# NVIDIA-ISAAC-ROS/isaac_ros_nvblox

Hardware: NVIDIA H100
Metric: depth-frames/sec (TSDF+ESDF integrate, 640x480 @ 5 cm voxels) (higher is better)
Workload: dtype f32

## Files before the change

### isaac_ros_nvblox_b200/csrc/nvb_api.cu

```cuda
#include <algorithm>
#include <array>
#include <cfloat>
#include <cmath>
#include <cstdio>
#include <cstring>
#include <set>
#include <string>
#include <vector>

#include "nvb_internal.cuh"

using namespace nvb;

namespace {

thread_local std::string g_last_error;

int fail(int code, const std::string& msg) {
  g_last_error = msg;
  return code;
}

#define NVB_CUDA(expr)                                                                               \
  do {                                                                                               \
// ... 315 lines not shown
  N.count = L->count;
  N.free_count = L->free_count;
  NVB_CUDA(cudaMalloc(&N.free_slots, (size_t)new_capacity * sizeof(int)));
  NVB_CUDA(cudaMemcpyAsync(N.free_slots, L->free_slots, (size_t)L->capacity * sizeof(int), cudaMemcpyDeviceToDevice,
                           m->stream));
  N.capacity = new_capacity;
  N.block_bytes = L->block_bytes;
  NVB_CUDA(cudaMalloc(&N.blocks, (size_t)new_capacity * L->block_bytes));
  NVB_CUDA(cudaMemsetAsync(N.blocks, 0, (size_t)new_capacity * L->block_bytes, m->stream));
  NVB_CUDA(cudaMemcpyAsync(N.blocks, L->blocks, (size_t)count * L->block_bytes, cudaMemcpyDeviceToDevice, m->stream));
  NVB_CUDA(cudaMalloc(&N.block_index, (size_t)new_capacity * 3 * sizeof(int)));
  NVB_CUDA(cudaMemcpyAsync(N.block_index, L->block_index, (size_t)count * 3 * sizeof(int), cudaMemcpyDeviceToDevice,
                           m->stream));
  const int hcap = nextPow2(2ll * new_capacity);
  N.hash.mask = (unsigned int)hcap - 1;
  NVB_CUDA(cudaMalloc(&N.hash.keys, (size_t)hcap * sizeof(unsigned long long)));
  NVB_CUDA(cudaMalloc(&N.hash.vals, (size_t)hcap * sizeof(int)));
  launchFillU64(N.hash.keys, kEmptyKey, (size_t)hcap, m->stream);
  launchRehash(N, count, m->stream);
  NVB_CUDA(syncAll(m));
  cudaFree(L->blocks), cudaFree(L->block_index), cudaFree(L->hash.keys), cudaFree(L->hash.vals), cudaFree(L->free_slots);
  *L = N;
  return NVB_OK;
}

int allocWaveXRecords(NvbMapper* m, int cap) {
  const int grid = esdfWaveXGrid(m->num_sms, m->esdf_reserved_sms);
  NVB_CUDA(syncAll(m));
  if (m->xrec) cudaFree(m->xrec);
  m->xrec = nullptr;
  m->xseg = 6 * ((cap + grid - 1) / grid) + 64;
  m->xseg_grid = grid;
  NVB_CUDA(cudaMalloc(&m->xrec, 2 * (size_t)grid * m->xseg * 32 * sizeof(int)));
  return NVB_OK;
}

int allocEsdfScratch(NvbMapper* m, int old_cap, int cap) {
  int rc;
  if ((rc = reallocCopy(&m->work, 0, (size_t)cap, false, m->stream))) return rc;
  if ((rc = reallocCopy(&m->upd_list, 0, (size_t)cap, false, m->stream))) return rc;
  if ((rc = reallocCopy(&m->clr_list, 0, (size_t)cap, false, m->stream))) return rc;
  if ((rc = reallocCopy(&m->clr_cand, 0, (size_t)cap, false, m->stream))) return rc;
  if ((rc = reallocCopy(&m->cleared_list, (size_t)old_cap, (size_t)cap, true, m->stream))) return rc;
  if ((rc = reallocCopy(&m->ring_a, 0, (size_t)cap, false, m->stream))) return rc;
  if ((rc = reallocCopy(&m->ring_b, 0, (size_t)cap, false, m->stream))) return rc;
  if ((rc = reallocCopy(&m->stamp_a, (size_t)old_cap, (size_t)cap, true, m->stream))) return rc;
  if ((rc = reallocCopy(&m->stamp_b, (size_t)old_cap, (size_t)cap, true, m->stream))) return rc;
  if ((rc = reallocCopy(&m->seed_upd, (size_t)old_cap, (size_t)cap, true, m->stream))) return rc;
  if ((rc = reallocCopy(&m->seed_clr, (size_t)old_cap, (size_t)cap, true, m->stream))) return rc;
  if ((rc = reallocCopy(&m->psum, 2 * (size_t)old_cap, 2 * (size_t)cap, true, m->stream))) return rc;
  {
    int* q = nullptr;
    NVB_CUDA(cudaMalloc(&q, (size_t)cap * 6 * sizeof(int)));
    NVB_CUDA(cudaMemsetAsync(q, 0xFE, (size_t)cap * 6 * sizeof(int), m->stream));
    if (m->nbr && old_cap)
      NVB_CUDA(cudaMemcpyAsync(q, m->nbr, (size_t)old_cap * 6 * sizeof(int), cudaMemcpyDeviceToDevice, m->stream));
    NVB_CUDA(syncAll(m));
    if (m->nbr) cudaFree(m->nbr);
    m->nbr = q;
  }
  {
    int* q = nullptr;
    NVB_CUDA(cudaMalloc(&q, (size_t)cap * 27 * sizeof(int)));
    NVB_CUDA(cudaMemsetAsync(q, 0xFE, (size_t)cap * 27 * sizeof(int), m->stream));
    if (m->nbr27 && old_cap)
      NVB_CUDA(cudaMemcpyAsync(q, m->nbr27, (size_t)old_cap * 27 * sizeof(int), cudaMemcpyDeviceToDevice, m->stream));
    NVB_CUDA(syncAll(m));
    if (m->nbr27) cudaFree(m->nbr27);
    m->nbr27 = q;
  }
  if ((rc = reallocCopy(&m->cand_stamp, (size_t)old_cap, (size_t)cap, true, m->stream))) return rc;
  if ((rc = reallocCopy(&m->cand_a, 0, (size_t)cap, false, m->stream))) return rc;
  if ((rc = reallocCopy(&m->cand_b, 0, (size_t)cap, false, m->stream))) return rc;
  if (m->esdf_persistent == 2) {
    if (m->shadow) cudaFree(m->shadow);
    m->shadow = nullptr;
    NVB_CUDA(cudaMalloc(&m->shadow, (size_t)cap * kEsdfBlockBytes));
    m->shadow_cap = cap;
  }
  if (m->esdf_persistent == 3) {
    NVB_CUDA(syncAll(m));
    if (m->xslab) cudaFree(m->xslab);
    m->xslab = nullptr;
    NVB_CUDA(cudaMalloc(&m->xslab, 2 * (size_t)cap * kEsdfBlockBytes));
    int rc;
    if ((rc = allocWaveXRecords(m, cap))) return rc;
    if (!m->xcounts) {
      NVB_CUDA(cudaMalloc(&m->xcounts, esdfWaveXFlagBytes()));
      NVB_CUDA(cudaMemsetAsync(m->xcounts, 0, esdfWaveXFlagBytes(), m->stream));
    }
  }
  return NVB_OK;
}

int allocTsdfSide(NvbMapper* m, int old_cap, int cap) {
  int rc;
  if ((rc = reallocCopy(&m->dirty, (size_t)old_cap, (size_t)cap, true, m->stream))) return rc;
  if ((rc = reallocCopy(&m->todo_slots, (size_t)old_cap, (size_t)cap, true, m->stream))) return rc;
  if (m->projective_layer_type == NVB_PROJECTIVE_TSDF_WITH_FREESPACE) {
    if ((rc = reallocCopy(&m->dirty_fs, (size_t)old_cap, (size_t)cap, true, m->stream))) return rc;
    if ((rc = reallocCopy(&m->todo_fs_slots, (size_t)old_cap, (size_t)cap, true, m->stream))) return rc;
  }
  if (m->dirty_mesh) {
    if ((rc = reallocCopy(&m->dirty_mesh, (size_t)old_cap, (size_t)cap, true, m->stream))) return rc;
    if ((rc = reallocCopy(&m->todo_mesh_slots, (size_t)old_cap, (size_t)cap, true, m->stream))) return rc;
  }
  return NVB_OK;
}

constexpr int kHostListCap = 1 << 15;

enum { kWorkCount = 0, kUpdCount = 1, kClrCount = 2, kClrAabb = 3, kClearedCount = 9, kRingCount = 10, kRingId = 14,
       kTodoCount = 15, kFrameCount = 16, kError = 17, kClearedSeq = 18, kTailState = 20, kDeadCount = 22, kDeadClearedCount = 23, kGesCounts = 24, kTodoFsCount = 28, kFsWorkCount = 29, kColsCount = 30, kColorWorkCount = 31, kXTail = 32, kTodoMeshCount = 36, kClrCandCount = 37, kNumInts = 40 };

float logOddsFromProbability(float p);

EsdfCtx makeEsdfCtx(NvbMapper* m) {
  EsdfCtx c{};
  c.tsdf = m->tsdf, c.esdf = m->esdf;
  c.freespace = m->freespace;
  c.use_freespace = m->projective_layer_type == NVB_PROJECTIVE_TSDF_WITH_FREESPACE ? 1 : 0;
  c.work = m->work;
  c.work_count = m->esdf_ints + kWorkCount;
  c.upd_list = m->upd_list, c.upd_count = m->esdf_ints + kUpdCount;
  c.clr_list = m->clr_list, c.clr_count = m->esdf_ints + kClrCount;
  c.clr_cand = m->clr_cand, c.clr_cand_count = m->esdf_ints + kClrCandCount;
  c.clr_aabb = m->esdf_ints + kClrAabb;
  c.cleared_list = m->cleared_list, c.cleared_count = m->esdf_ints + kClearedCount;
  c.ring_a = m->ring_a, c.ring_b = m->ring_b;
  c.ring_count = m->esdf_ints + kRingCount;
  c.tail_state = m->esdf_ints + kTailState;
  c.stamp_a = m->stamp_a, c.stamp_b = m->stamp_b;
  c.ring_id = m->esdf_ints + kRingId;
  c.nbr = m->nbr, c.seed_upd = m->seed_upd, c.seed_clr = m->seed_clr;
  c.clr_bits = m->clr_bits;
  c.psum = m->psum, c.prune = (m->prune_ok && m->esdf_persistent == 3) ? 1 : 0;
  c.nbr27 = m->nbr27, c.shadow = m->shadow, c.cand_stamp = m->cand_stamp;
  c.xslab = m->xslab, c.xrec = m->xrec, c.xtail = m->esdf_ints + kXTail, c.xseg = m->xseg, c.xcounts = m->xcounts;
  c.xsplit_min_k = m->esdf_split_min_k;
  c.ges_counts = m->esdf_ints + kGesCounts;
  c.cand_a = m->cand_a, c.cand_b = m->cand_b, c.ges_switch = m->ges_switch;
  c.colset_keys = m->colset, c.colset_mask = m->colset_n ? (unsigned int)(m->colset_n - 1) : 0u;
  c.cols = m->cols, c.cols_count = m->esdf_ints + kColsCount;
  c.dead_cleared_xyz = m->dead_cleared_xyz;
  c.dead_cleared_count = m->dead_cleared_xyz ? m->esdf_ints + kDeadClearedCount : nullptr;
  c.cleared_seq = m->esdf_ints + kClearedSeq;
  c.update_seq = m->update_seq;
  c.barrier = m->barrier;
  c.phase_max = m->phase_max;
  c.stats = m->stats;
  c.error = m->error_dev;
  const float max_esdf_distance_vox = m->ep.max_esdf_distance_m / m->voxel_size;
  c.max_sq = max_esdf_distance_vox * max_esdf_distance_vox;
  c.max_esdf_distance_m = m->ep.max_esdf_distance_m;
  c.max_site_distance_m = m->ep.max_site_distance_vox * m->voxel_size;
  c.min_weight = m->ep.min_weight;
  c.block_size = m->block_size;
  c.from_occupancy = m->projective_layer_type == NVB_PROJECTIVE_OCCUPANCY ? 1 : 0;
  c.occupied_threshold_log_odds = logOddsFromProbability(m->ep.occupied_threshold);
  return c;
}

float logOddsFromProbability(float p) {
  p = fmaxf(1e-3f, fminf(p, 1.0f - 1e-3f));
  return logf(p / (1.0f - p));
}

// ... 2987 lines not shown
```

### isaac_ros_nvblox_b200/csrc/nvb_esdf_wavex.cu

```cuda
#include "nvb_esdf_wave_common.cuh"

#include <cstdlib>

namespace nvb {

namespace {

#ifndef NVB_WAVEX_THREADS
#define NVB_WAVEX_THREADS 512
#endif
#ifndef NVB_WAVEX_MAXREG
#define NVB_WAVEX_MAXREG 96
#endif
#ifndef NVB_WAVEX_TAIL
#define NVB_WAVEX_TAIL 1
#endif
#ifndef NVB_WAVEX_PROF
#define NVB_WAVEX_PROF 0
#endif
#ifndef NVB_WAVEX_SPEC_HALO
#define NVB_WAVEX_SPEC_HALO 0
#endif
#if NVB_WAVEX_PROF
#define X_PROF_BEGIN() long long tq = clock64();
#define X_PROF(i) \
  if (lane64 == 0) xs.prof[group][i] += clock64() - tq; \
  tq = clock64();
#define X_PROF_COUNT(i) \
  if (lane64 == 0) xs.prof[group][i]++;
#define X_PROF_BIN(i, j, K)                                                  \
  if (lane64 == 0) {                                                         \
    const int kb = (K) <= 256 ? 0 : ((K) <= 1040 ? 1 : 2);                   \
    const long long dt = clock64() - tq;                                     \
    xs.prof[group][i] += dt, xs.prof[group][(j) + kb] += dt, xs.prof[group][(j) + 3 + kb]++; \
  }                                                                          \
  tq = clock64();
#else
#define X_PROF_BEGIN()
#define X_PROF(i)
#define X_PROF_COUNT(i)
#define X_PROF_BIN(i, j, K)
#endif
constexpr int kXT = NVB_WAVEX_THREADS;
constexpr int kXG = kXT / 64;
constexpr int kRecInts = 32;
constexpr int kMaxCtas = 192;
constexpr int kRX = 110, kRY = 11;
constexpr int kRegionVox = 1100;
constexpr int kFlagBase = 4 * kRegionVox;
constexpr int kXRegionWords = 5 * kRegionVox;
constexpr size_t kXSmemBytes = (size_t)kXG * kXRegionWords * sizeof(unsigned int);

struct XTables {
  unsigned int halo[8][64];
  unsigned int pair[6][4][64];
};

struct XShared {
  int rec[kXG][kRecInts];
  int nb[kXG][8];
  int pos[kXG][8];
  unsigned int mask[kXG];
  int changed[kXG];
  unsigned int live[kXG][8];
  int seg[kXG][2];
  int pre[kMaxCtas + 1];
  int warp_tot[2][8];
  int ncand, nchanged;
  int next;
  int cur[kXG];
  int seeds[kXG];
  int bcast[4];
  unsigned int generation;
  int n_bar;
  int ring;
  int swept, faces, rings, n_tail;
  int n_split, n_rest;
#if NVB_WAVEX_PROF
  long long prof[kXG][16];
#endif
};

struct XCtx {
  unsigned char* blocks;
  int* block_index;
  DevHash hash;
  int* nbr;
  int* nbr27;
  int* cand_stamp;
  unsigned int* psum;
  int* stamp[2];
  unsigned char* X[2];
  int* recs[2];
  int seg;
  int split_min_k;
  int* error;
  float max_sq;
  __device__ __forceinline__ int* segment(int p, int cta) const { return recs[p] + (size_t)cta * seg * kRecInts; }
};

__shared__ XTables x_tab;
__shared__ XShared x_xs;
__shared__ XCtx x_ctx;
extern __shared__ __align__(16) unsigned int x_smem[];

__device__ __forceinline__ int rvox(int rx, int ry, int rz) { return rx * kRX + ry * kRY + rz; }
__device__ __forceinline__ int faceEntry(int f) {
  return f == 0 ? 22 : (f == 1 ? 4 : (f == 2 ? 16 : (f == 3 ? 10 : (f == 4 ? 14 : 12))));
}
__device__ __forceinline__ int boundaryOff(int r) { return r == 0 ? -1 : (r == 9 ? 1 : 0); }
__device__ __forceinline__ int boundaryLoc(int r) { return r == 0 ? 7 : (r == 9 ? 0 : r - 1); }

__device__ __forceinline__ int neighbor27(const XCtx& c, int slot, int d) {
  int v = __ldcg(c.nbr27 + 27 * slot + d);
  if (v < -1) {
    const int* bi = c.block_index + 3 * slot;
    v = (d == 13) ? slot : hashFind(c.hash, bi[0] + d / 9 - 1, bi[1] + (d / 3) % 3 - 1, bi[2] + d % 3 - 1);
    c.nbr27[27 * slot + d] = v;
  }
  return v;
}
__device__ __forceinline__ int neighbor6(const XCtx& c, int slot, int dir) {
  int v = __ldcg(c.nbr + 6 * slot + dir);
  if (v < -1) {
    const int* bi = c.block_index + 3 * slot;
    const int d = (dir & 1) ? -1 : 1;
    v = hashFind(c.hash, bi[0] + ((dir >> 1) == 0 ? d : 0), bi[1] + ((dir >> 1) == 1 ? d : 0), bi[2] + ((dir >> 1) == 2 ? d : 0));
    c.nbr[6 * slot + dir] = v;
  }
  return v;
}

__device__ __forceinline__ void initTables(XTables& tab, int tid) {
  for (int i = tid; i < 512; i += kXT) {
    const int k = i >> 6, lane = i & 63;
    unsigned int e = 0;
    int ra = 1, r1 = 1, r2 = 1, axis = 0;
    bool valid = true;
    if (k < 6) {
      axis = k >> 1;
      ra = (k & 1) ? 0 : 9, r1 = (lane >> 3) + 1, r2 = (lane & 7) + 1;
    } else {
      const int n = i - 384;
      if (n < 96) {
        const int edge = n >> 3, cn = edge & 3;
        axis = edge >> 2;
        ra = (n & 7) + 1, r1 = (cn & 1) ? 9 : 0, r2 = (cn & 2) ? 9 : 0;
      } else if (n < 104) {
        const int cn = n - 96;
        ra = (cn & 1) ? 9 : 0, r1 = (cn & 2) ? 9 : 0, r2 = (cn & 4) ? 9 : 0;
      } else {
        valid = false;
      }
    }
    if (valid) {
      const int rx = axis == 0 ? ra : r1, ry = axis == 0 ? r1 : (axis == 1 ? ra : r2), rz = axis == 2 ? ra : r2;
      const int d = (boundaryOff(rx) + 1) * 9 + (boundaryOff(ry) + 1) * 3 + (boundaryOff(rz) + 1);
      e = (unsigned)rvox(rx, ry, rz) | ((unsigned)(boundaryLoc(rx) * 64 + boundaryLoc(ry) * 8 + boundaryLoc(rz)) << 11) |
          ((unsigned)d << 20) | (1u << 25);
    }
    tab.halo[k][lane] = e;
  }
  for (int i = tid; i < 6 * 4 * 64; i += kXT) {
    const int pass = i >> 8, j = (i >> 6) & 3, lane = i & 63;
    const int axis = pass >> 1, dir = (pass & 1) ? -1 : 1;
    int plane, u, w;
    bool valid = true;
    if (j < 2) {
      plane = j, u = (lane >> 3) + 1, w = (lane & 7) + 1;
    } else {
      const int n = (j - 2) * 64 + lane;
      plane = n / 36;
      const int q = n % 36;
      if (q < 10) u = 0, w = q;
      else if (q < 20) u = 9, w = q - 10;
      else if (q < 28) u = q - 20 + 1, w = 0;
      else u = q - 28 + 1, w = 9;
      if (n >= 72) valid = false, plane = 0, u = 1, w = 1;
    }
    unsigned int e = 0;
    if (valid) {
      const int sa = dir > 0 ? (plane ? 8 : 0) : (plane ? 9 : 1);
      const int so = dir > 0 ? (plane ? 0 : -1) : (plane ? 1 : 0);
      const int da = sa + dir;
      const int A = axis == 0 ? 9 : (axis == 1 ? 3 : 1), U = axis == 0 ? 3 : 9, W = axis == 2 ? 3 : 1;
      const int d = 13 + so * A + boundaryOff(u) * U + boundaryOff(w) * W;
      const int inner = da >= 1 && da <= 8 && u >= 1 && u <= 8 && w >= 1 && w <= 8;
      const int sv = axis == 0 ? rvox(sa, u, w) : (axis == 1 ? rvox(u, sa, w) : rvox(u, w, sa));
      const int dv = axis == 0 ? rvox(da, u, w) : (axis == 1 ? rvox(u, da, w) : rvox(u, w, da));
      e = (unsigned)sv | ((unsigned)dv << 11) | ((unsigned)d << 22) | ((unsigned)inner << 27) | (1u << 28);
    }
    tab.pair[pass][j][lane] = e;
  }
}

struct LiveMasks {
  unsigned int* live;
  unsigned int needed;
  unsigned int axes;
};
__device__ __forceinline__ LiveMasks liveMasks(unsigned int mask, unsigned int* live_smem, bool writer) {
  LiveMasks L;
  L.live = live_smem;
  const unsigned int ok = mask | (1u << 13);
  const unsigned int D[6] = {0x7FFFE00u, 0x3FE00u, 0x3F000u, 0x7000u, 0x6000u, 0x2000u};
  unsigned int acc = 0;
  L.axes = 0;
#pragma unroll
  for (int p = 0; p < 6; p++) {
    const int axis = p >> 1;
    const int A = axis == 0 ? 9 : (axis == 1 ? 3 : 1);
    const unsigned int lo = axis == 0 ? 0x000001ffu : (axis == 1 ? 0x001c0e07u : 0x01249249u);
    const unsigned int dst_ok = ok & D[p];
    unsigned int lv, dst;
    if ((p & 1) == 0) {
      lv = mask & (lo | (lo << A)) & (dst_ok >> A);
      dst = lv << A;
    } else {
      lv = mask & ((lo << A) | (lo << (2 * A))) & (dst_ok << A);
      dst = lv >> A;
    }
    if (writer) live_smem[p] = lv;
    if (lv) L.axes |= 1u << axis;
    acc |= lv | dst;
  }
  L.needed = acc & mask & ~(1u << 13);
  return L;
}

struct OwnRegs {
  uint4 q[10];
};
__device__ __forceinline__ OwnRegs ownLoad(const unsigned char* blk, int lane64) {
  OwnRegs o;
  const uint4* src = reinterpret_cast<const uint4*>(blk) + lane64 * 10;
#pragma unroll
  for (int i = 0; i < 10; i++) o.q[i] = __ldcg(src + i);
  return o;
}
__device__ __forceinline__ unsigned int liveAxes(const unsigned int* live) {
  return ((live[0] | live[1]) ? 1u : 0u) | ((live[2] | live[3]) ? 2u : 0u) | ((live[4] | live[5]) ? 4u : 0u);
}
__device__ __forceinline__ unsigned int ownWord(const OwnRegs& o, int w) {
  const uint4& v = o.q[w >> 2];
  return (w & 3) == 0 ? v.x : ((w & 3) == 1 ? v.y : ((w & 3) == 2 ? v.z : v.w));
}
__device__ __forceinline__ void ownToShared(unsigned int* R, const OwnRegs& o, int lane64) {
  uint4* A = reinterpret_cast<uint4*>(R);
  const int v0 = rvox((lane64 >> 3) + 1, (lane64 & 7) + 1, 1);
#pragma unroll
  for (int z = 0; z < 8; z++) {
    A[v0 + z] = make_uint4(ownWord(o, 5 * z), ownWord(o, 5 * z + 1), ownWord(o, 5 * z + 2), ownWord(o, 5 * z + 3));
    R[kFlagBase + v0 + z] = ownWord(o, 5 * z + 4);
  }
}
__device__ __forceinline__ void ownStore(unsigned char* layer_blk, bool to_layer, unsigned char* x_blk, const unsigned int* R,
                                         unsigned int* psum_slot, int lane64) {
  const uint4* A = reinterpret_cast<const uint4*>(R);
  const int x = lane64 >> 3, y = lane64 & 7;
  const int v0 = rvox(x + 1, y + 1, 1);
  uint4* dl = reinterpret_cast<uint4*>(layer_blk) + lane64 * 10;
  uint4* dx = reinterpret_cast<uint4*>(x_blk) + lane64 * 10;
  int lo0 = 99, lo1 = 99, lo2 = 99, hi0 = -99, hi1 = -99, hi2 = -99;
#pragma unroll
  for (int h = 0; h < 2; h++) {
    unsigned int w[20];
#pragma unroll
    for (int z = 0; z < 4; z++) {
      const uint4 a = A[v0 + 4 * h + z];
      w[5 * z] = a.x, w[5 * z + 1] = a.y, w[5 * z + 2] = a.z, w[5 * z + 3] = a.w;
      w[5 * z + 4] = R[kFlagBase + v0 + 4 * h + z];
      if ((a.y | a.z | a.w) != 0u) {
        const int b0 = (x + (int)a.y) >> 3, b1 = (y + (int)a.z) >> 3, b2 = (4 * h + z + (int)a.w) >> 3;
        lo0 = min(lo0, b0), hi0 = max(hi0, b0), lo1 = min(lo1, b1), hi1 = max(hi1, b1), lo2 = min(lo2, b2), hi2 = max(hi2, b2);
      }
    }
#pragma unroll
    for (int i = 0; i < 5; i++) {
      const uint4 v = make_uint4(w[4 * i], w[4 * i + 1], w[4 * i + 2], w[4 * i + 3]);
      if (to_layer) __stcg(dl + 5 * h + i, v);
      __stcg(dx + 5 * h + i, v);
    }
  }
  if (psum_slot) {
    lo0 = __reduce_min_sync(0xffffffffu, lo0), lo1 = __reduce_min_sync(0xffffffffu, lo1), lo2 = __reduce_min_sync(0xffffffffu, lo2);
    hi0 = __reduce_max_sync(0xffffffffu, hi0), hi1 = __reduce_max_sync(0xffffffffu, hi1), hi2 = __reduce_max_sync(0xffffffffu, hi2);
    if ((lane64 & 31) == 0) {
      unsigned int v = 0u;
      if (lo0 <= hi0) {
        const bool fits = lo0 >= -16 && lo1 >= -16 && lo2 >= -16 && hi0 <= 15 && hi1 <= 15 && hi2 <= 15;
        v = fits ? ((1u << 31) | (unsigned)(lo0 + 16) | ((unsigned)(hi0 + 16) << 5) | ((unsigned)(lo1 + 16) << 10) |
                    ((unsigned)(hi1 + 16) << 15) | ((unsigned)(lo2 + 16) << 20) | ((unsigned)(hi2 + 16) << 25))
                 : 0xffffffffu;
      }
      psum_slot[lane64 >> 5] = v;
    }
  }
}

__device__ __forceinline__ void cpAsync4(unsigned int* smem_dst, const unsigned int* gsrc) {
  asm volatile("cp.async.ca.shared.global [%0], [%1], 4;" ::"r"((unsigned int)__cvta_generic_to_shared(smem_dst)), "l"(gsrc)
               : "memory");
}
__device__ __forceinline__ void ownAsync(unsigned int* R, const unsigned char* blk, int lane64, unsigned int axes, bool planes) {
  const int y = lane64 >> 3, z = lane64 & 7;
  const bool lane_on = ((axes & 2u) && (y == 0 || y == 7)) || ((axes & 4u) && (z == 0 || z == 7));
  const unsigned int* src = reinterpret_cast<const unsigned int*>(blk) + lane64 * kEsdfVoxelWords;
  const int v0 = rvox(1, y + 1, z + 1);
#pragma unroll
  for (int x = 0; x < 8; x++) {
    const bool on = lane_on || ((axes & 1u) && (x == 0 || x == 7));
    if (on == planes) {
      const unsigned int* s = src + x * 64 * kEsdfVoxelWords;
      const int v = v0 + x * kRX;
#pragma unroll
      for (int w = 0; w < 4; w++) cpAsync4(R + 4 * v + w, s + w);
      cpAsync4(R + kFlagBase + v, s + 4);
    }
  }
}
__device__ __forceinline__ void haloAsync(const XTables& tab, unsigned int* R, const int* row, const unsigned char* X, int lane64,
                                          unsigned int batches, unsigned int blocks) {
#pragma unroll 1
  while (batches) {
    const int k = __ffs(batches) - 1;
    batches &= batches - 1;
    const unsigned int e = tab.halo[k][lane64];
    const int d = (e >> 20) & 31u;
    const int slot = ((e >> 25) & 1u) && ((blocks >> d) & 1u) ? row[d] : -1;
    if (slot >= 0) {
      const unsigned int* src = reinterpret_cast<const unsigned int*>(X + (size_t)slot * kEsdfBlockBytes) + ((e >> 11) & 511u) * kEsdfVoxelWords;
      const int v = e & 2047u;
#pragma unroll
      for (int w = 0; w < 4; w++) cpAsync4(R + 4 * v + w, src + w);
      cpAsync4(R + kFlagBase + v, src + 4);
    }
  }
}
constexpr unsigned int kFaceBlocks = (1u << 22) | (1u << 4) | (1u << 16) | (1u << 10) | (1u << 14) | (1u << 12);
__device__ __forceinline__ unsigned int haloBatches(unsigned int needed) {
  unsigned int bl = ((needed >> 22) & 1u) | (((needed >> 4) & 1u) << 1) | (((needed >> 16) & 1u) << 2) | (((needed >> 10) & 1u) << 3) |
                    (((needed >> 14) & 1u) << 4) | (((needed >> 12) & 1u) << 5);
  if (needed & ~kFaceBlocks) bl |= 0xC0u;
  return bl;
}

__device__ __forceinline__ bool replayX(const XTables& tab, unsigned int* R, const LiveMasks& L, int lane64, int group,
                                        float max_sq) {
  uint4* A = reinterpret_cast<uint4*>(R);
  const unsigned int* live_p = L.live;
  bool changed = false;
#pragma unroll 1
  for (int pass = 0; pass < 6; pass++) {
    const unsigned int live = live_p[pass];
    if (!live) continue;
    const int axis = pass >> 1, dir = (pass & 1) ? -1 : 1;
    const int s0 = axis == 0 ? dir : 0, s1 = axis == 1 ? dir : 0, s2 = axis == 2 ? dir : 0;
#pragma unroll 1
    for (int j = 0; j < 4; j++) {
      unsigned int e = tab.pair[pass][j][lane64];
      if (!((e >> 28) & 1u) || !((live >> ((e >> 22) & 31u)) & 1u)) e = 0;
      if (__any_sync(0xffffffffu, e != 0u)) {
        const int sv = e & 2047u, dv = (e >> 11) & 2047u;
        const uint4 es = A[sv], ns = A[dv];
        const unsigned int ef = R[kFlagBase + sv], nf = R[kFlagBase + dv];
        const bool ok = e != 0u && flagObserved(ef) && flagObserved(nf) && !flagSite(nf) && !(__uint_as_float(es.x) >= max_sq);
        const int d0 = (int)es.y - s0, d1 = (int)es.z - s1, d2 = (int)es.w - s2;
        const float pdist = (float)(d0 * d0 + (d1 * d1 + d2 * d2));
        if (ok && __uint_as_float(ns.x) > pdist) {
          A[dv] = make_uint4(__float_as_uint(pdist), (unsigned)d0, (unsigned)d1, (unsigned)d2);
          changed = changed || ((e >> 27) & 1u);
        }
      }
    }
    groupSync(group);
  }
  return changed;
}

template <int AXIS>
__device__ __forceinline__ bool sweepLineX(unsigned int* R, int a, int b, float max_sq) {
  uint4* A = reinterpret_cast<uint4*>(R);
  const int v0 = AXIS == 0 ? rvox(1, a + 1, b + 1) : (AXIS == 1 ? rvox(a + 1, 1, b + 1) : rvox(a + 1, b + 1, 1));
  constexpr int stride = AXIS == 0 ? kRX : (AXIS == 1 ? kRY : 1);
  constexpr int kNone = 1 << 28, kCap = 1 << 27;
  int T[kVps], pa[kVps], po1[kVps], po2[kVps], pp2[kVps];
  unsigned int tk = 0, dirty = 0;
#pragma unroll
  for (int i = 0; i < kVps; i++) {
    const uint4 q = A[v0 + i * stride];
    const unsigned int fl = R[kFlagBase + v0 + i * stride];
    const float sq = __uint_as_float(q.x);
    const bool o = flagObserved(fl), st = flagSite(fl);
    const int t = min(__float2int_ru(sq), kCap);
    T[i] = (o && !st) ? t : INT_MIN;
    const int qa = (int)(AXIS == 0 ? q.y : (AXIS == 1 ? q.z : q.w));
    const int q1 = (int)(AXIS == 0 ? q.z : q.y);
    const int q2 = (int)(AXIS == 2 ? q.z : q.w);
    pa[i] = st ? 0 : qa, po1[i] = st ? 0 : q1, po2[i] = st ? 0 : q2;
    pp2[i] = po1[i] * po1[i] + po2[i] * po2[i];
    if (o && (st || sq < max_sq)) tk |= 1u << i;
  }
#pragma unroll
  for (int pass = 0; pass < 2; pass++) {
    int la = 0, lo1 = 0, lo2 = 0, lp2 = kNone;
#pragma unroll
    for (int kk = 0; kk < kVps; kk++) {
      const int k = pass ? (kVps - 1 - kk) : kk;
      const int t = la - k;
      const int pd = t * t + lp2;
      const bool improve = T[k] > pd;
      const bool take = ((tk >> k) & 1u) && !improve;
      const int offer_a = pa[k] + k;
      if (improve) {
        T[k] = pd, pa[k] = t, po1[k] = lo1, po2[k] = lo2, pp2[k] = lp2;
        dirty |= 1u << k;
      }
      la = take ? offer_a : la;
// ... 41 lines not shown
    const int idx = lane64 + 64 * k;
    s.v[k] = -1;
    if (idx < 162) {
      const int nb = xs.nb[group][idx / 27];
      if (nb >= 0) s.v[k] = __ldcg(c.nbr27 + 27 * nb + idx % 27);
    }
  }
  return s;
}
__device__ __forceinline__ void registerClaim(const XCtx& c, XShared& xs, RegState& s, int group, int lane64, int target) {
  if (lane64 < 32) {
    const bool win = lane64 < 6 && xs.nb[group][lane64] >= 0 && s.old != target;
    const unsigned int ballot = __ballot_sync(0xffffffffu, win);
    if (ballot) {
      int base = 0;
      if (lane64 == 0) base = atomicAdd(&xs.ncand, __popc(ballot));
      base = __shfl_sync(0xffffffffu, base, 0);
      if (win) s.pos = base + __popc(ballot & ((1u << lane64) - 1u));
      if (s.pos >= c.seg) {
        s.pos = -1;
        atomicOr(c.error, 8);
      }
    }
  }
}
__device__ __forceinline__ void registerFinish(const XCtx& c, XShared& xs, const RegState& s, int group, int lane64,
                                               int* segment) {
  if (lane64 < 6) xs.pos[group][lane64] = s.pos;
  groupSync(group);
#pragma unroll
  for (int k = 0; k < 3; k++) {
    const int idx = lane64 + 64 * k;
    if (idx < 162) {
      const int w = idx / 27, pos = xs.pos[group][w];
      if (pos >= 0) {
        int v = s.v[k];
        if (v < -1) v = neighbor27(c, xs.nb[group][w], idx % 27);
        __stcg(segment + (size_t)pos * kRecInts + 1 + idx % 27, v);
      }
    }
  }
  if (lane64 < 6 && s.pos >= 0) __stcg(segment + (size_t)s.pos * kRecInts, xs.nb[group][lane64]);
}

__device__ __noinline__ void processCandidate(int ring, int K) {
  const XCtx& c = x_ctx;
  const XTables& tab = x_tab;
  XShared& xs = x_xs;
  const int cta = blockIdx.x, group = threadIdx.x >> 6, lane64 = threadIdx.x & 63;
  unsigned int* R = x_smem + group * kXRegionWords;
  const int ci = ring & 1, ni = ci ^ 1;
  const bool split = K >= c.split_min_k;
  X_PROF_BEGIN()
  if (lane64 < 28) xs.rec[group][lane64] = __ldcg(c.segment(ci, xs.seg[group][0]) + (size_t)xs.seg[group][1] * kRecInts + lane64);
  groupSync(group);
  X_PROF(0)
  const int slot = xs.rec[group][0];
  const int* row = &xs.rec[group][1];
  const unsigned char* blk = c.blocks + (size_t)slot * kEsdfBlockBytes;
  int sv = ring - 1;
  if (lane64 < 27 && row[lane64] >= 0) sv = __ldcg(c.stamp[ci] + row[lane64]);
  if (NVB_WAVEX_SPEC_HALO) haloAsync(tab, R, row, c.X[ci], lane64, 0x3Fu, 0x7FFFFFFu);
  if (split) {
    const unsigned int m = __ballot_sync(0xffffffffu, lane64 < 27 && sv == ring);
    if (lane64 == 0) xs.mask[group] = m, xs.changed[group] = 0;
  } else {
    OwnRegs own = ownLoad(blk, lane64);
    const unsigned int m = __ballot_sync(0xffffffffu, lane64 < 27 && sv == ring);
    if (lane64 == 0) xs.mask[group] = m, xs.changed[group] = 0;
    ownToShared(R, own, lane64);
  }
  if (NVB_WAVEX_SPEC_HALO) cpAsyncWaitAll();
  groupSync(group);
  const LiveMasks L = liveMasks(xs.mask[group], xs.live[group], lane64 == 0);
  X_PROF_BIN(1, 9, K)
  const unsigned int rest = NVB_WAVEX_SPEC_HALO ? (L.needed & ~kFaceBlocks) : L.needed;
  if (split) {
    ownAsync(R, blk, lane64, L.axes, true);
    if (lane64 == 0) atomicAdd(&xs.n_split, 1);
  }
  if (rest) haloAsync(tab, R, row, c.X[ci], lane64, haloBatches(rest), rest);
  if (rest || split) cpAsyncWaitAll();
  groupSync(group);
  X_PROF(2)
  const bool ch = replayX(tab, R, L, lane64, group, c.max_sq);
  if (ch) xs.changed[group] = 1;
  groupSync(group);
  X_PROF(3)
  X_PROF_COUNT(6)
  if (xs.changed[group]) {
    if (lane64 < 6) xs.nb[group][lane64] = row[faceEntry(lane64)];
    if (lane64 == 0) {
      __stcg(c.stamp[ni] + slot, ring + 1);
      atomicAdd(&xs.nchanged, 1);
    }
    groupSync(group);
    if (split) ownAsync(R, blk, lane64, liveAxes(xs.live[group]), false);
    RegState rs = registerBegin(c, xs, group, lane64, ring + 1);
    if (split) {
      if (lane64 == 0) atomicAdd(&xs.n_rest, 1);
      cpAsyncWaitAll();
      groupSync(group);
    }
    X_PROF(8)
    sweepBlockX(R, group, lane64, c.max_sq);
    registerClaim(c, xs, rs, group, lane64, ring + 1);
    groupSync(group);
    X_PROF(4)
    ownStore(c.blocks + (size_t)slot * kEsdfBlockBytes, true, c.X[ni] + (size_t)slot * kEsdfBlockBytes, R, c.psum + 2 * (size_t)slot, lane64);
    registerFinish(c, xs, rs, group, lane64, c.segment(ni, cta));
    X_PROF_COUNT(7)
  }
  groupSync(group);
  X_PROF(5)
}

__device__ __noinline__ void processSeed(int ring, int slot) {
  const XCtx& c = x_ctx;
  XShared& xs = x_xs;
  const int cta = blockIdx.x, group = threadIdx.x >> 6, lane64 = threadIdx.x & 63;
  unsigned int* R = x_smem + group * kXRegionWords;
  const int ci = ring & 1;
  unsigned char* blk = c.blocks + (size_t)slot * kEsdfBlockBytes;
  OwnRegs own = ownLoad(blk, lane64);
  if (lane64 < 6) xs.nb[group][lane64] = neighbor6(c, slot, lane64);
  if (lane64 == 0) {
    __stcg(c.stamp[ci] + slot, ring);
    xs.changed[group] = 0;
  }
  groupSync(group);
  RegState rs = registerBegin(c, xs, group, lane64, ring);
  ownToShared(R, own, lane64);
  groupSync(group);
  const bool ch = sweepBlockX(R, group, lane64, c.max_sq);
  registerClaim(c, xs, rs, group, lane64, ring);
  if (ch) xs.changed[group] = 1;
  groupSync(group);
  ownStore(blk, xs.changed[group] != 0, c.X[ci] + (size_t)slot * kEsdfBlockBytes, R, xs.changed[group] ? c.psum + 2 * (size_t)slot : nullptr, lane64);
  registerFinish(c, xs, rs, group, lane64, c.segment(ci, cta));
  groupSync(group);
}

#ifndef NVB_WAVEX_BARRIER_RA
#define NVB_WAVEX_BARRIER_RA 1
#endif
__device__ __forceinline__ void gridBarrierRA(unsigned int* bar, unsigned int& generation, unsigned int nctas) {
  __syncthreads();
  if (threadIdx.x == 0) {
    generation++;
    const unsigned int target = generation * nctas;
    asm volatile("red.release.gpu.global.add.u32 [%0], 1;" ::"l"(bar) : "memory");
    unsigned int v;
    do {
      asm volatile("ld.acquire.gpu.global.u32 %0, [%1];" : "=r"(v) : "l"(bar) : "memory");
    } while (v < target);
  }
  __syncthreads();
}

__device__ __forceinline__ void counterBarrierScan(XShared& xs, unsigned int* bar, unsigned int& generation, int2* counts, int nctas,
                                                   int cta, int tid, int seg, int ring_inc, int* K, int* M) {
  counts += (xs.n_bar & 1) * kMaxCtas;
  __syncthreads();
  if (tid == 0) {
    __stcg(counts + cta, make_int2(min(xs.ncand, seg), xs.nchanged));
    xs.ncand = 0, xs.nchanged = 0;
  }
  if (NVB_WAVEX_BARRIER_RA)
    gridBarrierRA(bar, generation, nctas);
  else
    gridBarrier(bar, generation, nctas);
  int2 v = make_int2(0, 0);
  if (tid < nctas) v = __ldcg(counts + tid);
  const int lane = tid & 31, warp = tid >> 5;
  int inc = v.x, chg = v.y;
#pragma unroll
  for (int o = 1; o < 32; o <<= 1) {
    const int t = __shfl_up_sync(0xffffffffu, inc, o);
    if (lane >= o) inc += t;
  }
#pragma unroll
  for (int o = 16; o > 0; o >>= 1) chg += __shfl_xor_sync(0xffffffffu, chg, o);
  if (warp < 8 && lane == 31) xs.warp_tot[0][warp] = inc;
  if (warp < 8 && lane == 0) xs.warp_tot[1][warp] = chg;
  __syncthreads();
  int base = 0, mtot = 0;
#pragma unroll
  for (int w = 0; w < 8; w++) {
    if (w < warp) base += xs.warp_tot[0][w];
    if (w * 32 < nctas) mtot += xs.warp_tot[1][w];
  }
  if (tid < nctas) xs.pre[tid + 1] = base + inc;
  if (tid == 0) xs.pre[0] = 0, xs.next = 0, xs.ring += ring_inc, xs.n_bar++;
  __syncthreads();
  *K = xs.pre[nctas];
  *M = mtot;
}

__global__ void __maxnreg__(NVB_WAVEX_MAXREG) esdfWaveXKernel(EsdfCtx c) {
  XShared& xs = x_xs;
  const int cta = blockIdx.x, nctas = gridDim.x;
  const int tid = threadIdx.x, group = tid >> 6, lane64 = tid & 63;
  if (*(volatile int*)c.work_count == 0) return;
  initTables(x_tab, tid);
  if (tid == 0) {
    xs.ncand = 0, xs.nchanged = 0, xs.next = 0;
    xs.ring = *(volatile int*)c.ring_id;
    xs.generation = 0, xs.n_bar = 0, xs.swept = 0, xs.faces = 0, xs.rings = 0, xs.n_tail = 0, xs.n_split = 0, xs.n_rest = 0;
    XCtx& xc = x_ctx;
    xc.blocks = c.esdf.blocks, xc.block_index = c.esdf.block_index, xc.hash = c.esdf.hash;
    xc.nbr = c.nbr, xc.nbr27 = c.nbr27, xc.cand_stamp = c.cand_stamp, xc.psum = c.psum;
    xc.stamp[0] = c.stamp_a, xc.stamp[1] = c.stamp_b;
    xc.X[0] = c.xslab, xc.X[1] = c.xslab + (size_t)c.esdf.capacity * kEsdfBlockBytes;
    xc.recs[0] = c.xrec, xc.recs[1] = c.xrec + (size_t)nctas * c.xseg * kRecInts;
    xc.seg = c.xseg, xc.split_min_k = c.xsplit_min_k, xc.error = c.error, xc.max_sq = c.max_sq;
  }
#if NVB_WAVEX_PROF
  if (lane64 < 16) xs.prof[group][lane64] = 0;
#endif
  __syncthreads();
#if NVB_WAVEX_PROF
  long long t_bar = 0, t_work = 0, t0 = globalTimerNs(), t1;
  int dbgK = 0, dbgM = 0;
#define X_DBG(k, m) dbgK = (k), dbgM = (m);
#define X_TIME_WORK()                                                                                                      \
  t1 = globalTimerNs(), t_work += t1 - t0;                                                                                 \
  if (tid == 0 && xs.n_bar < 1000) atomicMax((unsigned long long*)c.phase_max + xs.n_bar, (unsigned long long)(t1 - t0)); \
  if (cta == 0 && tid == 0 && xs.n_bar < 1000)                                                                             \
    c.phase_max[1000 + xs.n_bar] = dbgK, c.phase_max[2000 + xs.n_bar] = dbgM, c.phase_max[3000 + xs.n_bar] = t1 - t0;      \
  t0 = t1;
#define X_TIME_BARRIER() t1 = globalTimerNs(), t_bar += t1 - t0, t0 = t1;
#else
#define X_DBG(k, m)
#define X_TIME_WORK()
#define X_TIME_BARRIER()
#endif
#define X_BARRIER(inc, Kout, Mout)                                                                                        \
  X_TIME_WORK()                                                                                                           \
  counterBarrierScan(xs, c.barrier, xs.generation, reinterpret_cast<int2*>(c.xcounts), nctas, cta, tid, c.xseg, inc,        \
                     &(Kout), &(Mout));                                                                                   \
  X_TIME_BARRIER()
  for (int pass = 0; pass < 2; pass++) {
    const int* src = pass ? c.cleared_list : c.upd_list;
    const int n0 = pass ? *(volatile int*)c.cleared_count : *(volatile int*)c.upd_count;
    if (n0 == 0) continue;
    X_DBG(-1, n0)
    if (lane64 == 0) xs.seeds[group] = n0;
    for (;;) {
      if (lane64 == 0) xs.cur[group] = atomicAdd(&xs.next, 1);
      groupSync(group);
      const long long e = (long long)cta + (long long)xs.cur[group] * nctas;
      if (e >= xs.seeds[group]) break;
      processSeed(xs.ring, __ldcg(src + e));
    }
    int M = xs.seeds[group], K, unused;
    X_BARRIER(0, K, unused)
    if (tid == 0) xs.swept += M;
    while (true) {
      X_DBG(K, M)
      if (NVB_WAVEX_TAIL && K <= kXG) {
        if (cta == 0) {
          int t = 0;
          if (group < K) {
            for (int s = lane64; s < nctas; s += 64)
              if (xs.pre[s] <= group && group < xs.pre[s + 1]) xs.seg[group][0] = s, xs.seg[group][1] = group - xs.pre[s];
          }
          __syncthreads();
          while (true) {
            if (group < K) processCandidate(xs.ring, -1);
            __syncthreads();
            const int K2 = min(xs.ncand, c.xseg), M2 = xs.nchanged;
            __syncthreads();
            if (tid == 0) xs.ncand = 0, xs.nchanged = 0, xs.faces += 6 * M, xs.rings++, xs.swept += M2, xs.ring++;
            if (tid < kXG) xs.seg[tid][0] = 0, xs.seg[tid][1] = tid;
            t++;
            M = M2, K = K2;
            __syncthreads();
            if (M == 0 || K > kXG) break;
          }
          if (tid == 0) xs.n_tail += t, c.xtail[0] = t, c.xtail[1] = K, c.xtail[2] = M;
        }
        {
          int k_unused, m_unused;
          X_BARRIER(0, k_unused, m_unused)
        }
        if (cta != 0) {
          if (tid == 0) xs.bcast[0] = __ldcg(c.xtail + 0), xs.bcast[1] = __ldcg(c.xtail + 1), xs.bcast[2] = __ldcg(c.xtail + 2);
          __syncthreads();
          K = xs.bcast[1], M = xs.bcast[2];
          if (tid == 0) xs.ring += xs.bcast[0];
          __syncthreads();
        }
        if (M == 0) break;
        for (int s = tid; s <= nctas; s += kXT) xs.pre[s] = s == 0 ? 0 : K;
        __syncthreads();
        continue;
      }
      for (;;) {
        if (lane64 == 0) xs.cur[group] = atomicAdd(&xs.next, 1);
        groupSync(group);
        const long long e = (long long)cta + (long long)xs.cur[group] * nctas;
        if (e >= K) break;
        for (int s = lane64; s < nctas; s += 64)
          if (xs.pre[s] <= e && e < xs.pre[s + 1]) xs.seg[group][0] = s, xs.seg[group][1] = (int)e - xs.pre[s];
        groupSync(group);
        processCandidate(xs.ring, K);
      }
      int K2, M2;
      X_BARRIER(1, K2, M2)
      if (tid == 0) xs.faces += 6 * M, xs.rings++, xs.swept += M2;
      M = M2, K = K2;
      if (M == 0) break;
    }
    if (tid == 0) xs.ring++;
    __syncthreads();
  }
#undef X_BARRIER
#undef X_TIME_WORK
#undef X_TIME_BARRIER
#undef X_DBG
  if (tid == 0 && xs.n_split) {
    atomicAdd((unsigned long long*)&c.stats[14], (unsigned long long)xs.n_split);
    atomicAdd((unsigned long long*)&c.stats[15], (unsigned long long)xs.n_rest);
  }
  if (cta == 0 && tid == 0) {
    *c.ring_id = xs.ring + 1;
    c.stats[4] = *(volatile int*)c.cleared_count;
    c.stats[5] = xs.swept, c.stats[6] = xs.faces, c.stats[7] = xs.rings;
    c.stats[10] = xs.n_tail, c.stats[11] = xs.n_bar;
#if NVB_WAVEX_PROF
    c.stats[8] = t_bar, c.stats[9] = t_work;
    long long sum_max = 0;
    for (int q = 0; q < xs.n_bar && q < 1000; q++) sum_max += (long long)c.phase_max[q];
    c.stats[12] = sum_max;
    for (int q = 0; q < 16; q++) c.phase_max[3984 + q] = xs.prof[0][q];
#endif
  }
}

}

int esdfWaveXGrid(int num_sms, int reserved_sms) {
  int grid = num_sms < kMaxCtas ? num_sms : kMaxCtas;
  if (reserved_sms > 0 && grid - reserved_sms >= 8) grid -= reserved_sms;
  return grid;
}
size_t esdfWaveXFlagBytes() { return 2 * (size_t)kMaxCtas * sizeof(int2); }

constexpr int kSplitMinK = 0;
int esdfWaveXSplitMinK() {
  const char* e = getenv("NVB_WAVEX_SPLIT_MIN_K");
  const int v = e ? atoi(e) : kSplitMinK;
  return v < 0 ? 0 : v;
}

cudaError_t launchEsdfComputeX(const EsdfCtx& c, int num_sms, int reserved_sms, cudaStream_t stream, int* launches) {
  static int per_sm = -1;
  if (per_sm < 0) {
    cudaFuncSetAttribute(esdfWaveXKernel, cudaFuncAttributeMaxDynamicSharedMemorySize, (int)kXSmemBytes);
    int v = 0;
    if (cudaOccupancyMaxActiveBlocksPerMultiprocessor(&v, esdfWaveXKernel, kXT, kXSmemBytes) != cudaSuccess) v = 0;
    per_sm = v;
  }
  if (per_sm <= 0) return cudaErrorLaunchOutOfResources;
  EsdfCtx cc = c;
  void* args[] = {&cc};
  (*launches)++;
  const int grid = esdfWaveXGrid(num_sms, reserved_sms);
  return cudaLaunchCooperativeKernel((const void*)esdfWaveXKernel, dim3(grid), dim3(kXT), args, kXSmemBytes, stream);
}

}
```

### isaac_ros_nvblox_b200/csrc/nvb_internal.cuh

```cuda
#pragma once
#include <cstdint>

#include <cuda_runtime.h>
#include <stdint.h>

#include "nvblox_b200.h"

namespace nvb {

constexpr int kVps = 8;
constexpr int kVpb = kVps * kVps * kVps;
constexpr int kTsdfBlockBytes = kVpb * 8;
constexpr int kEsdfBlockBytes = kVpb * 20;
constexpr int kEsdfVoxelWords = 5;
constexpr int kColorBlockBytes = kVpb * 8;
constexpr int kOccBlockBytes = kVpb * 4;
constexpr int kHelperCtas = 132;

struct Vec3 {
  float x, y, z;
};

struct Rigid {
  float r[3][3];
// ... 274 lines not shown
                              const Rigid& T_C_L, const NvbCamera& cam, const TsdfKernelParams& p,
                              const OccKernelParams& op, int num_sms, unsigned int* bits_to_clear, int num_words,
                              cudaStream_t stream);

struct EsdfCtx {
  DevLayer tsdf;
  DevLayer esdf;
  DevLayer freespace;
  int use_freespace;
  int4* work;
  int* work_count;
  int* upd_list;
  int* upd_count;
  int* clr_list;
  int* clr_count;
  int* clr_aabb;
  int* cleared_list;
  int* cleared_count;
  int* ring_a;
  int* ring_b;
  int* ring_count;
  int* tail_state;
  int* stamp_a;
  int* stamp_b;
  int* ring_id;
  int* nbr;
  int* nbr27;
  unsigned char* shadow;
  unsigned char* xslab;
  int* xtail;
  int* xrec;
  int xseg;
  int xsplit_min_k;
  int* xcounts;
  int slice_mode;
  int slice_min_bz, slice_min_vz, slice_max_bz, slice_max_vz, slice_out_bz, slice_out_vz;
  int slice_planar;
  float plane_nx, plane_ny, plane_nz, plane_d, slice_above_plane_m, slice_thickness_m;
  unsigned long long* colset_keys;
  unsigned int colset_mask;
  int* cols;
  int* cols_count;
  int* dead_cleared_xyz;
  int* dead_cleared_count;
  int* cand_a;
  int* cand_b;
  int ges_switch;
  int* cand_stamp;
  int* ges_counts;
  unsigned int* psum;
  int* clr_cand;
  int* clr_cand_count;
  unsigned int* clr_bits;
  int prune;
  int* seed_upd;
  int* seed_clr;
  int* cleared_seq;
  int update_seq;
  int* tracker_dirty;
  int* tracker_todo_count;
  unsigned int* barrier;
  unsigned long long* phase_max;
  long long* stats;
  int* error;
  float max_sq;
  float max_esdf_distance_m;
  float max_site_distance_m;
  float min_weight;
  float block_size;
  int from_occupancy;
  float occupied_threshold_log_odds;
};
void launchEsdfSliceAllocateAndMark(const EsdfCtx& c, const int* in_xyz, const int* in_slots, const int* in_count_dev,
                                    int in_count_upper, int num_sms, cudaStream_t stream);
void launchEsdfAllocate(const EsdfCtx& c, const int* in_xyz, const int* in_slots, const int* in_count_dev,
                        int in_count_upper, cudaStream_t stream);
void launchEsdfMark(const EsdfCtx& c, int count_upper, int num_sms, cudaStream_t stream);
int launchEsdfClear(const EsdfCtx& c, int esdf_count_upper, int num_sms, cudaStream_t stream);
cudaError_t launchEsdfComputeGes(const EsdfCtx& c, int num_sms, cudaStream_t stream, int* launches);
cudaError_t launchEsdfComputePersistent(const EsdfCtx& c, int num_sms, cudaStream_t stream, int* launches);
cudaError_t launchEsdfComputeX(const EsdfCtx& c, int num_sms, int reserved_sms, cudaStream_t stream, int* launches);
int esdfWaveXGrid(int num_sms, int reserved_sms);
size_t esdfWaveXFlagBytes();
int esdfWaveXSplitMinK();
cudaError_t runEsdfComputeHostLoop(const EsdfCtx& c, int num_sms, cudaStream_t stream, int* launches);
int esdfPersistentMaxCtas(int num_sms);

constexpr int kFreespaceVoxelBytes = 24;
constexpr int kFreespaceBlockBytes = 512 * kFreespaceVoxelBytes;
struct FreespaceArgs {
  DevLayer tsdf, fs;
  const int* todo_slots;
  const int* todo_count;
  const int* in_xyz;
  int n_explicit;
  int* tracker_dirty;
  int4* work;
  int* work_count;
  int* error;
  float max_tsdf_distance_for_occupancy_m;
  long long max_unobserved_ms, min_free_ms, min_reset_ms;
  int check_neighborhood, init_high_confidence;
  long long last_update_ms, now_ms;
  const float* depth;
  int rows, cols;
  Rigid T_C_L;
  NvbCamera cam;
  TsdfKernelParams p;
};
void launchFreespaceUpdate(const FreespaceArgs& a, int upper, int num_sms, cudaStream_t stream);

struct MarkFreeArgs {
  DevLayer layer;
  int occupancy;
  int3 lo, size;
  int cells;
  float cx, cy, cz, radius, block_size, trunc_m;
  int4* out;
  int* out_count;
  int* error;
  int *dirty, *todo_slots, *todo_count;
  int *dirty2, *todo2_slots, *todo2_count;
  int *dirty3, *todo3_slots, *todo3_count;
};
void launchMarkFreeSphere(const MarkFreeArgs& a, int num_sms, cudaStream_t stream);

struct ColorArgs {
  DevLayer tsdf, color;
  Rigid T_C_L, T_L_C;
  NvbCamera cam;
  int3 aabb_lo, aabb_hi;
  float vmin_x, vmin_y, vmax_x, vmax_y;
  float block_size, voxel_size, half_voxel_size, voxel_size_inv;
  float trunc_m, max_integration_distance_m, max_weight, measurement_weight;
  float w_old_h, w_new_h;
  int4* work;
  int* work_count;
  int* error;
  float* synth;
  int drows, dcols, subsample, depth_subsample;
  int max_steps;
  float max_ray_len, eps_m;
  const unsigned char* color_image;
  const unsigned char* mask;
  int mask_mode;
  int rows, cols;
};
void launchColorSelect(const ColorArgs& a, int num_sms, cudaStream_t stream);
void launchSphereTrace(const ColorArgs& a, cudaStream_t stream);
void launchColorIntegrate(const ColorArgs& a, int num_sms, cudaStream_t stream);

struct DecayArgs {
  DevLayer layer;
  int occupancy;
  float decay_factor, weight_threshold, free_distance_m;
  int set_free_distance;
  float free_log_odds, occupied_log_odds, to_log_odds;
  int deallocate;
  const int* skip_stamp;
  int skip_seq;
  int has_sphere;
  float cx, cy, cz, r2;
  const float* depth;
  int rows, cols;
  Rigid T_C_L;
  NvbCamera cam;
// ... 133 lines not shown
```

Measured before the change: 2811.

## Store only boundary face cells in wave-X exchange slab with 16-byte halo loads

The cross-block exchange slab (X) now holds only the six boundary faces of each block, as 16-byte distance cells plus separate flag words, rather than a full copy of the ESDF block. ownStore writes just those face cells, and haloAsync fetches each neighbour cell with a single 16-byte cp.async.cg instead of four 4-byte copies. This shrinks slab memory and global write/read traffic per propagated block. The halo table now encodes a face-cell index instead of a voxel index, and the candidate loop bound uses xs.pre[nctas] rather than K; profiling bins were also extended.

```diff
diff --git a/isaac_ros_nvblox_b200/csrc/nvb_api.cu b/isaac_ros_nvblox_b200/csrc/nvb_api.cu
--- a/isaac_ros_nvblox_b200/csrc/nvb_api.cu
+++ b/isaac_ros_nvblox_b200/csrc/nvb_api.cu
@@ -421,7 +421,7 @@
     NVB_CUDA(syncAll(m));
     if (m->xslab) cudaFree(m->xslab);
     m->xslab = nullptr;
-    NVB_CUDA(cudaMalloc(&m->xslab, 2 * (size_t)cap * kEsdfBlockBytes));
+    NVB_CUDA(cudaMalloc(&m->xslab, esdfWaveXSlabBytes(cap)));
     int rc;
     if ((rc = allocWaveXRecords(m, cap))) return rc;
     if (!m->xcounts) {
diff --git a/isaac_ros_nvblox_b200/csrc/nvb_esdf_wavex.cu b/isaac_ros_nvblox_b200/csrc/nvb_esdf_wavex.cu
--- a/isaac_ros_nvblox_b200/csrc/nvb_esdf_wavex.cu
+++ b/isaac_ros_nvblox_b200/csrc/nvb_esdf_wavex.cu
@@ -35,11 +35,19 @@
     xs.prof[group][i] += dt, xs.prof[group][(j) + kb] += dt, xs.prof[group][(j) + 3 + kb]++; \
   }                                                                          \
   tq = clock64();
+#define X_PROF_KBIN(i, j, K)                                \
+  if (lane64 == 0) {                                        \
+    const int kb = (K) <= 256 ? 0 : ((K) <= 1040 ? 1 : 2);  \
+    const long long dt = clock64() - tq;                    \
+    xs.prof[group][i] += dt, xs.prof[group][(j) + kb] += dt; \
+  }                                                         \
+  tq = clock64();
 #else
 #define X_PROF_BEGIN()
 #define X_PROF(i)
 #define X_PROF_COUNT(i)
 #define X_PROF_BIN(i, j, K)
+#define X_PROF_KBIN(i, j, K)
 #endif
 constexpr int kXT = NVB_WAVEX_THREADS;
 constexpr int kXG = kXT / 64;
@@ -50,6 +58,13 @@
 constexpr int kFlagBase = 4 * kRegionVox;
 constexpr int kXRegionWords = 5 * kRegionVox;
 constexpr size_t kXSmemBytes = (size_t)kXG * kXRegionWords * sizeof(unsigned int);
+constexpr int kXFaceCells = 6 * 64;
+constexpr int kXFlagOff = kXFaceCells * 16;
+constexpr int kXSlotBytes = kXFaceCells * (16 + 4);
+#if NVB_WAVEX_PROF
+constexpr int kXProfWords = 24;
+constexpr int kXProfBase = 4000 - kXProfWords;
+#endif
 
 struct XTables {
   unsigned int halo[8][64];
@@ -77,7 +92,7 @@
   int swept, faces, rings, n_tail;
   int n_split, n_rest;
 #if NVB_WAVEX_PROF
-  long long prof[kXG][16];
+  long long prof[kXG][kXProfWords];
 #endif
 };
 
@@ -136,15 +151,16 @@
     const int k = i >> 6, lane = i & 63;
     unsigned int e = 0;
     int ra = 1, r1 = 1, r2 = 1, axis = 0;
+    int fa = 0;
     bool valid = true;
     if (k < 6) {
-      axis = k >> 1;
+      axis = k >> 1, fa = axis;
       ra = (k & 1) ? 0 : 9, r1 = (lane >> 3) + 1, r2 = (lane & 7) + 1;
     } else {
       const int n = i - 384;
       if (n < 96) {
         const int edge = n >> 3, cn = edge & 3;
-        axis = edge >> 2;
+        axis = edge >> 2, fa = axis == 0 ? 1 : 0;
         ra = (n & 7) + 1, r1 = (cn & 1) ? 9 : 0, r2 = (cn & 2) ? 9 : 0;
       } else if (n < 104) {
         const int cn = n - 96;
@@ -156,8 +172,10 @@
     if (valid) {
       const int rx = axis == 0 ? ra : r1, ry = axis == 0 ? r1 : (axis == 1 ? ra : r2), rz = axis == 2 ? ra : r2;
       const int d = (boundaryOff(rx) + 1) * 9 + (boundaryOff(ry) + 1) * 3 + (boundaryOff(rz) + 1);
-      e = (unsigned)rvox(rx, ry, rz) | ((unsigned)(boundaryLoc(rx) * 64 + boundaryLoc(ry) * 8 + boundaryLoc(rz)) << 11) |
-          ((unsigned)d << 20) | (1u << 25);
+      const int lx = boundaryLoc(rx), ly = boundaryLoc(ry), lz = boundaryLoc(rz);
+      const int lf = fa == 0 ? lx : (fa == 1 ? ly : lz), l1 = fa == 0 ? ly : lx, l2 = fa == 2 ? ly : lz;
+      const int cell = (2 * fa + (lf == 0 ? 1 : 0)) * 64 + l1 * 8 + l2;
+      e = (unsigned)rvox(rx, ry, rz) | ((unsigned)cell << 11) | ((unsigned)d << 20) | (1u << 25);
     }
     tab.halo[k][lane] = e;
   }
@@ -254,13 +272,21 @@
     R[kFlagBase + v0 + z] = ownWord(o, 5 * z + 4);
   }
 }
-__device__ __forceinline__ void ownStore(unsigned char* layer_blk, bool to_layer, unsigned char* x_blk, const unsigned int* R,
+__device__ __forceinline__ void ownStore(unsigned char* layer_blk, bool to_layer, unsigned char* x_slot, const unsigned int* R,
                                          unsigned int* psum_slot, int lane64) {
   const uint4* A = reinterpret_cast<const uint4*>(R);
   const int x = lane64 >> 3, y = lane64 & 7;
   const int v0 = rvox(x + 1, y + 1, 1);
   uint4* dl = reinterpret_cast<uint4*>(layer_blk) + lane64 * 10;
-  uint4* dx = reinterpret_cast<uint4*>(x_blk) + lane64 * 10;
+  uint4* xc = reinterpret_cast<uint4*>(x_slot) + lane64;
+  unsigned int* xf = reinterpret_cast<unsigned int*>(x_slot + kXFlagOff) + lane64;
+#pragma unroll
+  for (int f = 0; f < 6; f++) {
+    const int fa = f >> 1, p = (f & 1) ? 1 : 8;
+    const int v = fa == 0 ? rvox(p, x + 1, y + 1) : (fa == 1 ? rvox(x + 1, p, y + 1) : rvox(x + 1, y + 1, p));
+    __stcg(xc + f * 64, A[v]);
+    __stcg(xf + f * 64, R[kFlagBase + v]);
+  }
   int lo0 = 99, lo1 = 99, lo2 = 99, hi0 = -99, hi1 = -99, hi2 = -99;
 #pragma unroll
   for (int h = 0; h < 2; h++) {
@@ -276,11 +302,8 @@
       }
     }
 #pragma unroll
-    for (int i = 0; i < 5; i++) {
-      const uint4 v = make_uint4(w[4 * i], w[4 * i + 1], w[4 * i + 2], w[4 * i + 3]);
-      if (to_layer) __stcg(dl + 5 * h + i, v);
-      __stcg(dx + 5 * h + i, v);
-    }
+    for (int i = 0; i < 5; i++)
+      if (to_layer) __stcg(dl + 5 * h + i, make_uint4(w[4 * i], w[4 * i + 1], w[4 * i + 2], w[4 * i + 3]));
   }
   if (psum_slot) {
     lo0 = __reduce_min_sync(0xffffffffu, lo0), lo1 = __reduce_min_sync(0xffffffffu, lo1), lo2 = __reduce_min_sync(0xffffffffu, lo2);
@@ -302,6 +325,10 @@
   asm volatile("cp.async.ca.shared.global [%0], [%1], 4;" ::"r"((unsigned int)__cvta_generic_to_shared(smem_dst)), "l"(gsrc)
                : "memory");
 }
+__device__ __forceinline__ void cpAsyncCell(unsigned int* smem_dst, const void* gsrc) {
+  asm volatile("cp.async.cg.shared.global [%0], [%1], 16;" ::"r"((unsigned int)__cvta_generic_to_shared(smem_dst)), "l"(gsrc)
+               : "memory");
+}
 __device__ __forceinline__ void ownAsync(unsigned int* R, const unsigned char* blk, int lane64, unsigned int axes, bool planes) {
   const int y = lane64 >> 3, z = lane64 & 7;
   const bool lane_on = ((axes & 2u) && (y == 0 || y == 7)) || ((axes & 4u) && (z == 0 || z == 7));
@@ -329,11 +356,10 @@
     const int d = (e >> 20) & 31u;
     const int slot = ((e >> 25) & 1u) && ((blocks >> d) & 1u) ? row[d] : -1;
     if (slot >= 0) {
-      const unsigned int* src = reinterpret_cast<const unsigned int*>(X + (size_t)slot * kEsdfBlockBytes) + ((e >> 11) & 511u) * kEsdfVoxelWords;
-      const int v = e & 2047u;
-#pragma unroll
-      for (int w = 0; w < 4; w++) cpAsync4(R + 4 * v + w, src + w);
-      cpAsync4(R + kFlagBase + v, src + 4);
+      const unsigned char* xslot = X + (size_t)slot * kXSlotBytes;
+      const int cell = (e >> 11) & 511u, v = e & 2047u;
+      cpAsyncCell(R + 4 * v, xslot + 16 * cell);
+      cpAsync4(R + kFlagBase + v, reinterpret_cast<const unsigned int*>(xslot + kXFlagOff) + cell);
     }
   }
 }
@@ -541,7 +567,7 @@
   if (rest) haloAsync(tab, R, row, c.X[ci], lane64, haloBatches(rest), rest);
   if (rest || split) cpAsyncWaitAll();
   groupSync(group);
-  X_PROF(2)
+  X_PROF_KBIN(2, 15, K)
   const bool ch = replayX(tab, R, L, lane64, group, c.max_sq);
   if (ch) xs.changed[group] = 1;
   groupSync(group);
@@ -566,12 +592,12 @@
     registerClaim(c, xs, rs, group, lane64, ring + 1);
     groupSync(group);
     X_PROF(4)
-    ownStore(c.blocks + (size_t)slot * kEsdfBlockBytes, true, c.X[ni] + (size_t)slot * kEsdfBlockBytes, R, c.psum + 2 * (size_t)slot, lane64);
+    ownStore(c.blocks + (size_t)slot * kEsdfBlockBytes, true, c.X[ni] + (size_t)slot * kXSlotBytes, R, c.psum + 2 * (size_t)slot, lane64);
     registerFinish(c, xs, rs, group, lane64, c.segment(ni, cta));
     X_PROF_COUNT(7)
   }
   groupSync(group);
-  X_PROF(5)
+  X_PROF_KBIN(5, 18, K)
 }
 
 __device__ __noinline__ void processSeed(int ring, int slot) {
@@ -595,7 +621,7 @@
   registerClaim(c, xs, rs, group, lane64, ring);
   if (ch) xs.changed[group] = 1;
   groupSync(group);
-  ownStore(blk, xs.changed[group] != 0, c.X[ci] + (size_t)slot * kEsdfBlockBytes, R, xs.changed[group] ? c.psum + 2 * (size_t)slot : nullptr, lane64);
+  ownStore(blk, xs.changed[group] != 0, c.X[ci] + (size_t)slot * kXSlotBytes, R, xs.changed[group] ? c.psum + 2 * (size_t)slot : nullptr, lane64);
   registerFinish(c, xs, rs, group, lane64, c.segment(ci, cta));
   groupSync(group);
 }
@@ -670,12 +696,12 @@
     xc.blocks = c.esdf.blocks, xc.block_index = c.esdf.block_index, xc.hash = c.esdf.hash;
     xc.nbr = c.nbr, xc.nbr27 = c.nbr27, xc.cand_stamp = c.cand_stamp, xc.psum = c.psum;
     xc.stamp[0] = c.stamp_a, xc.stamp[1] = c.stamp_b;
-    xc.X[0] = c.xslab, xc.X[1] = c.xslab + (size_t)c.esdf.capacity * kEsdfBlockBytes;
+    xc.X[0] = c.xslab, xc.X[1] = c.xslab + (size_t)c.esdf.capacity * kXSlotBytes;
     xc.recs[0] = c.xrec, xc.recs[1] = c.xrec + (size_t)nctas * c.xseg * kRecInts;
     xc.seg = c.xseg, xc.split_min_k = c.xsplit_min_k, xc.error = c.error, xc.max_sq = c.max_sq;
   }
 #if NVB_WAVEX_PROF
-  if (lane64 < 16) xs.prof[group][lane64] = 0;
+  if (lane64 < kXProfWords) xs.prof[group][lane64] = 0;
 #endif
   __syncthreads();
 #if NVB_WAVEX_PROF
@@ -759,11 +785,11 @@
         if (lane64 == 0) xs.cur[group] = atomicAdd(&xs.next, 1);
         groupSync(group);
         const long long e = (long long)cta + (long long)xs.cur[group] * nctas;
-        if (e >= K) break;
+        if (e >= xs.pre[nctas]) break;
         for (int s = lane64; s < nctas; s += 64)
           if (xs.pre[s] <= e && e < xs.pre[s + 1]) xs.seg[group][0] = s, xs.seg[group][1] = (int)e - xs.pre[s];
         groupSync(group);
-        processCandidate(xs.ring, K);
+        processCandidate(xs.ring, xs.pre[nctas]);
       }
       int K2, M2;
       X_BARRIER(1, K2, M2)
@@ -792,7 +818,7 @@
     long long sum_max = 0;
     for (int q = 0; q < xs.n_bar && q < 1000; q++) sum_max += (long long)c.phase_max[q];
     c.stats[12] = sum_max;
-    for (int q = 0; q < 16; q++) c.phase_max[3984 + q] = xs.prof[0][q];
+    for (int q = 0; q < kXProfWords; q++) c.phase_max[kXProfBase + q] = xs.prof[0][q];
 #endif
   }
 }
@@ -805,6 +831,7 @@
   return grid;
 }
 size_t esdfWaveXFlagBytes() { return 2 * (size_t)kMaxCtas * sizeof(int2); }
+size_t esdfWaveXSlabBytes(int capacity) { return 2 * (size_t)capacity * kXSlotBytes; }
 
 constexpr int kSplitMinK = 0;
 int esdfWaveXSplitMinK() {
diff --git a/isaac_ros_nvblox_b200/csrc/nvb_internal.cuh b/isaac_ros_nvblox_b200/csrc/nvb_internal.cuh
--- a/isaac_ros_nvblox_b200/csrc/nvb_internal.cuh
+++ b/isaac_ros_nvblox_b200/csrc/nvb_internal.cuh
@@ -380,6 +380,7 @@
 cudaError_t launchEsdfComputeX(const EsdfCtx& c, int num_sms, int reserved_sms, cudaStream_t stream, int* launches);
 int esdfWaveXGrid(int num_sms, int reserved_sms);
 size_t esdfWaveXFlagBytes();
+size_t esdfWaveXSlabBytes(int capacity);
 int esdfWaveXSplitMinK();
 cudaError_t runEsdfComputeHostLoop(const EsdfCtx& c, int num_sms, cudaStream_t stream, int* launches);
 int esdfPersistentMaxCtas(int num_sms);
```

Measured after the change: 3148, median of 6. 12.0% higher.
